# mom-ocean/MOM6

Measured on AMD Instinct MI355X. Metric: simulated-days/wall-sec, higher is better.
Workload: dtype f64

## Files before the change

mom6_amd/csrc/barotropic.hip:

```cpp
#include <algorithm>
#include <type_traits>
#include <vector>
#include <cmath>
#include "mom6x_dev.h"


enum BTW {
  W_q = 0, W_DCor_u, W_DCor_v, W_gtot_E, W_gtot_W, W_gtot_N, W_gtot_S, W_eta, W_eta_PF,
  W_Cor_ref_u, W_Cor_ref_v, W_BT_force_u, W_BT_force_v, W_ubt, W_vbt, W_bt_rem_u, W_bt_rem_v,
  W_uhbt0, W_vhbt0, W_ubt_Cor, W_vbt_Cor, W_uhbt, W_vhbt, W_u_accel_bt, W_v_accel_bt,
  W_eta_src, W_e_anom, W_eta_sum, W_eta_wtd, W_ubt_wtd, W_vbt_wtd, W_eta_pred,
  W_uh0sum, W_vh0sum, W_ubt0, W_vbt0,
  W_f4u, W_f4u_2, W_f4u_3, W_f4u_4, W_f4v, W_f4v_2, W_f4v_3, W_f4v_4,
  W_BTCu,
  W_BTCv = W_BTCu + 10,
  W_BTtmp = W_BTCv + 10,
  W_uhn = W_BTtmp + 12,
  W_vhn,
  W_ubt2, W_vbt2, W_eta_pred2,
  W_COUNT
};

enum BTC { B_FA_EE = 0, B_FA_E0, B_FA_W0, B_FA_WW, B_uBT_WW, B_uBT_EE, B_crvW, B_crvE, B_uh_WW, B_uh_EE };

struct BTState {
  mom6x_barotropic_params P;
  double *frhatu, *frhatv, *IDatu, *IDatv, *ubtav, *vbtav, *eta_cor, *q_D, *D_u_Cor, *D_v_Cor;
  double *work;
  int nstep_last;
  unsigned long long *warn;
  double *warn_info;
  bool la_pending;
  const double *la_pbce;
  double la_underflow;
  bool fr_pending;
  const double *fr_hu, *fr_hv;
};

namespace {

__device__ __forceinline__ double *wp(double *work, const Dm &d, int m) { return work + (size_t)m * d.slab; }

__device__ __forceinline__ double find_uhbt(double u, const double *__restrict__ B, size_t c, size_t slab) {
  if (u == 0.0) return 0.0;
  const double uEE = B[B_uBT_EE * slab + c];
  if (u < uEE) return (u - uEE) * B[B_FA_EE * slab + c] + B[B_uh_EE * slab + c];
  if (u < 0.0) return u * (B[B_FA_E0 * slab + c] + B[B_crvE * slab + c] * (u * u));
  const double uWW = B[B_uBT_WW * slab + c];
  if (u <= uWW) return u * (B[B_FA_W0 * slab + c] + B[B_crvW * slab + c] * (u * u));
  return (u - uWW) * B[B_FA_WW * slab + c] + B[B_uh_WW * slab + c];
}

__global__ void k_bt_init_static(Dm d, const double *__restrict__ G, double Z_to_H, double Mean_SL,
                                 double cor_scale, double H_subroundoff, double *q_D, double *D_u_Cor,
                                 double *D_v_Cor, double *IDatu, double *IDatv) {
  const int i = -1 + blockIdx.x * blockDim.x + threadIdx.x;
  const int j = -1 + blockIdx.y * blockDim.y + threadIdx.y;
  if (i > d.ni - 1 || j > d.nj - 1) return;
  const int st = d.pitch;
  const size_t c = ix2(d, i, j);
  const double *bathyT = gm(G, d, MOM6X_G_bathyT), *areaT = gm(G, d, MOM6X_G_areaT), *mT = gm(G, d, MOM6X_G_mask2dT);
// ... 298 lines not shown
__global__ void k_btcl(Dm d, const double *__restrict__ tmp, double *Bu, double *Bv, int hs) {
  const int i = -hs - 1 + blockIdx.x * blockDim.x + threadIdx.x;
  const int j = -hs - 1 + blockIdx.y * blockDim.y + threadIdx.y;
  if (i > d.ni - 1 + hs || j > d.nj - 1 + hs) return;
  const size_t c = ix2(d, i, j), slab = (size_t)d.slab;
  const double C1_3 = 1.0 / 3.0;
  for (int dir = 0; dir < 2; dir++) {
    if (dir == 0 && j < -hs) continue;
    if (dir == 1 && i < -hs) continue;
    const double *t = tmp + (size_t)(dir * 6) * slab;
    double *B = dir ? Bv : Bu;
    const double FA_EE = t[2 * slab + c], FA_E0 = t[3 * slab + c], FA_W0 = t[4 * slab + c], FA_WW = t[5 * slab + c];
    const double uBT_EE = 1.0 * t[0 * slab + c], uBT_WW = 1.0 * t[1 * slab + c];
    B[B_FA_EE * slab + c] = FA_EE; B[B_FA_E0 * slab + c] = FA_E0; B[B_FA_W0 * slab + c] = FA_W0; B[B_FA_WW * slab + c] = FA_WW;
    B[B_uBT_EE * slab + c] = uBT_EE; B[B_uBT_WW * slab + c] = uBT_WW;
    B[B_uh_EE * slab + c] = uBT_EE * (C1_3 * (2.0 * FA_E0 + FA_EE));
    B[B_uh_WW * slab + c] = uBT_WW * (C1_3 * (2.0 * FA_W0 + FA_WW));
    double crvW = 0.0, crvE = 0.0;
    if (fabs(uBT_WW) > 0.0) crvW = (C1_3 * (FA_WW - FA_W0)) / (uBT_WW * uBT_WW);
    if (fabs(uBT_EE) > 0.0) crvE = (C1_3 * (FA_EE - FA_E0)) / (uBT_EE * uBT_EE);
    B[B_crvW * slab + c] = crvW; B[B_crvE * slab + c] = crvE;
  }
}

__global__ void k_uhbt0(Dm d, const double *__restrict__ work_c, double *work) {
  const int i = -1 + blockIdx.x * blockDim.x + threadIdx.x;
  const int j = -1 + blockIdx.y * blockDim.y + threadIdx.y;
  if (i > d.ni - 1 || j > d.nj - 1) return;
  const size_t c = ix2(d, i, j), slab = (size_t)d.slab;
  if (j >= 0) work[W_uhbt0 * slab + c] = work_c[W_uh0sum * slab + c] - find_uhbt(work_c[W_ubt0 * slab + c], work_c + W_BTCu * slab, c, slab);
  if (i >= 0) work[W_vhbt0 * slab + c] = work_c[W_vh0sum * slab + c] - find_uhbt(work_c[W_vbt0 * slab + c], work_c + W_BTCv * slab, c, slab);
}

__global__ void k_find_Cor(Dm d, double *work, int Sadourny, int isvf, int ievf, int jsvf, int jevf) {
  const int i = isvf - 1 + blockIdx.x * blockDim.x + threadIdx.x;
  const int j = jsvf - 1 + blockIdx.y * blockDim.y + threadIdx.y;
  if (i > ievf + 1 || j > jevf + 1) return;
  const int st = d.pitch;
  const size_t c = ix2(d, i, j), slab = (size_t)d.slab;
  const double *q = work + W_q * slab, *DCor_u = work + W_DCor_u * slab, *DCor_v = work + W_DCor_v * slab;
  double *f4u = work + W_f4u * slab, *f4v = work + W_f4v * slab;
  if (j <= jevf) {
    if (Sadourny) {
      f4v[0 * slab + c] = 1.0 * DCor_u[c - 1] * q[c - 1];
      f4v[1 * slab + c] = 1.0 * DCor_u[c] * q[c];
      f4v[3 * slab + c] = 1.0 * DCor_u[c + st] * q[c];
      f4v[2 * slab + c] = 1.0 * DCor_u[c - 1 + st] * q[c - 1];
    } else {
      f4v[0 * slab + c] = 1.0 * DCor_u[c - 1] * ((q[c] + q[c - 1 - st]) + q[c - 1]) / 3.0;
      f4v[1 * slab + c] = 1.0 * DCor_u[c] * (q[c] + (q[c - 1] + q[c - st])) / 3.0;
      f4v[3 * slab + c] = 1.0 * DCor_u[c + st] * (q[c] + (q[c - 1] + q[c + st])) / 3.0;
      f4v[2 * slab + c] = 1.0 * DCor_u[c - 1 + st] * ((q[c] + q[c - 1 + st]) + q[c - 1]) / 3.0;
    }
  }
  if (i <= ievf) {
    if (Sadourny) {
      f4u[3 * slab + c] = 1.0 * DCor_v[c + 1] * q[c];
      f4u[2 * slab + c] = 1.0 * DCor_v[c] * q[c];
      f4u[0 * slab + c] = 1.0 * DCor_v[c - st] * q[c - st];
      f4u[1 * slab + c] = 1.0 * DCor_v[c + 1 - st] * q[c - st];
    } else {
      f4u[3 * slab + c] = 1.0 * DCor_v[c + 1] * (q[c] + (q[c + 1] + q[c - st])) / 3.0;
      f4u[2 * slab + c] = 1.0 * DCor_v[c] * (q[c] + (q[c - 1] + q[c - st])) / 3.0;
      f4u[0 * slab + c] = 1.0 * DCor_v[c - st] * ((q[c] + q[c - 1 - st]) + q[c - st]) / 3.0;
      f4u[1 * slab + c] = 1.0 * DCor_v[c + 1 - st] * ((q[c] + q[c + 1 - st]) + q[c - st]) / 3.0;
    }
  }
}

__global__ void k_cor_ref_eta_src(Dm d, const double *__restrict__ G, double *work, double *eta_cor, double Instep,
                                  int bound_BT_corr, double maxCFL_Idt, double dt, double Z_to_H, double Z_ref, double maxvel) {
  const int i = -1 + blockIdx.x * blockDim.x + threadIdx.x;
  const int j = -1 + blockIdx.y * blockDim.y + threadIdx.y;
  if (i > d.ni - 1 || j > d.nj - 1) return;
  const int st = d.pitch;
  const size_t c = ix2(d, i, j), slab = (size_t)d.slab;
  const double *f4u = work + W_f4u * slab, *f4v = work + W_f4v * slab;
  const double *ubt_Cor = work + W_ubt_Cor * slab, *vbt_Cor = work + W_vbt_Cor * slab;
  if (j >= 0)
    work[W_Cor_ref_u * slab + c] = (((f4u[3 * slab + c] * vbt_Cor[c + 1]) + (f4u[0 * slab + c] * vbt_Cor[c - st])) +
                                    ((f4u[2 * slab + c] * vbt_Cor[c]) + (f4u[1 * slab + c] * vbt_Cor[c + 1 - st])));
  if (i >= 0)
    work[W_Cor_ref_v * slab + c] = -1.0 * (((f4v[0 * slab + c] * ubt_Cor[c - 1]) + (f4v[3 * slab + c] * ubt_Cor[c + st])) +
                                           ((f4v[1 * slab + c] * ubt_Cor[c]) + (f4v[2 * slab + c] * ubt_Cor[c - 1 + st])));
  if (i >= 0 && j >= 0) {
    const double mT = gm(G, d, MOM6X_G_mask2dT)[c];
    double ec = eta_cor[c];
    if (bound_BT_corr == 2) {
      const double *bathyT = gm(G, d, MOM6X_G_bathyT), *dy_Cu = gm(G, d, MOM6X_G_dy_Cu), *dx_Cv = gm(G, d, MOM6X_G_dx_Cv);
      auto Dat = [&](size_t a, size_t bb, double len) {
        const double H1 = (bathyT[a] + Z_ref) * Z_to_H, H2 = (bathyT[bb] + Z_ref) * Z_to_H;
        double D = 0.0;
        if ((H1 > 0.0) && (H2 > 0.0)) D = len * (2.0 * H1 * H2) / (H1 + H2);
        return D;
      };
      const double DatuW = Dat(c - 1, c, dy_Cu[c - 1]), DatuE = Dat(c, c + 1, dy_Cu[c]);
      const double DatvN = Dat(c, c + st, dx_Cv[c]), DatvS = Dat(c - st, c, dx_Cv[c - st]);
      const double bound = dt * (gm(G, d, MOM6X_G_IareaT)[c] * 0.1 * maxvel * ((DatuW + DatuE) + (DatvN + DatvS)));
      if (fabs(ec) > bound) ec = copysign(bound, ec);
      eta_cor[c] = ec;
    } else if (bound_BT_corr && mT > 0.0) {
      if (ec > 0.0) {
        const double u_max_cor = gm(G, d, MOM6X_G_dxT)[c] * maxCFL_Idt, v_max_cor = gm(G, d, MOM6X_G_dyT)[c] * maxCFL_Idt;
        const double *Bu = work + W_BTCu * slab, *Bv = work + W_BTCv * slab;
        const double *uhbt0 = work + W_uhbt0 * slab, *vhbt0 = work + W_vhbt0 * slab;
        const double eta_cor_max = dt * (gm(G, d, MOM6X_G_IareaT)[c] *
            (((find_uhbt(u_max_cor, Bu, c, slab) + uhbt0[c]) - (find_uhbt(-u_max_cor, Bu, c - 1, slab) + uhbt0[c - 1])) +
             ((find_uhbt(v_max_cor, Bv, c, slab) + vhbt0[c]) - (find_uhbt(-v_max_cor, Bv, c - st, slab) + vhbt0[c - st]))));
        ec = dmin(ec, dmax(0.0, eta_cor_max));
      } else {
        const double Htot = gm(G, d, MOM6X_G_bathyT)[c] * Z_to_H + work[W_eta * slab + c];
        ec = dmax(ec, -dmax(0.0, Htot));
      }
      eta_cor[c] = ec;
    }
    work[W_eta_src * slab + c] = mT * (Instep * ec);
  }
}

__global__ void k_bt_copy_in(Dm d, double *work, const double *__restrict__ eta_in, const double *__restrict__ eta_PF_in,
                             const double *__restrict__ q_D, const double *__restrict__ D_u_Cor,
                             const double *__restrict__ D_v_Cor) {
  const int i = -d.halo - 1 + blockIdx.x * blockDim.x + threadIdx.x;
  const int j = -d.halo - 1 + blockIdx.y * blockDim.y + threadIdx.y;
  if (i > d.ni - 1 + d.halo || j > d.nj - 1 + d.halo) return;
  const size_t c = ix2(d, i, j), slab = (size_t)d.slab;
  if (i >= -d.halo && j >= -d.halo) { work[W_eta * slab + c] = eta_in[c]; work[W_eta_PF * slab + c] = eta_PF_in[c]; }
  work[W_q * slab + c] = q_D[c]; work[W_DCor_u * slab + c] = D_u_Cor[c]; work[W_DCor_v * slab + c] = D_v_Cor[c];
}

struct LoopArgs {
  double dtbt, dgeo_de, vel_underflow, trans_wt1, trans_wt2;
  double wt_accel, wt_trans, wt_vel, wt_eta, wt_accel2;
  int project, bracket_bug, find_etaav;
  int f4_on_the_fly, Sadourny;
  int store_uhn, have_uhn;
  int pred_next;
  double wt_accel2_next;
  int isv, iev, jsv, jev;
};

__global__ void __launch_bounds__(256)
k_bt_pred(Dm d, const double *__restrict__ G, double *work, LoopArgs A, int p_ubt, int p_vbt, int p_pred, int sel) {
  const int i = I_BASE(A.isv - 1) + blockIdx.x * blockDim.x + threadIdx.x;
  const int j = A.jsv - 1 + blockIdx.y * blockDim.y + threadIdx.y;
  if (i < A.isv - 1 || i > A.iev + 1 || j > A.jev + 1) return;
  if (sel) { const bool own = (i >= 0 && i <= d.ni - 1 && j >= 0 && j <= d.nj - 1); if (own != (sel == 1)) return; }
  const int st = d.pitch;
  const size_t c = ix2(d, i, j), slab = (size_t)d.slab;
  double eta_PF_BT;
  if (A.project) {
    eta_PF_BT = work[W_eta * slab + c];
  } else {
    const double *ubt = work + (size_t)p_ubt * slab, *vbt = work + (size_t)p_vbt * slab;
    const double *Bu = work + W_BTCu * slab, *Bv = work + W_BTCv * slab;
    const double *uhbt0 = work + W_uhbt0 * slab, *vhbt0 = work + W_vhbt0 * slab;
    double uW, uE, vS, vN;
    if (A.have_uhn) {
      const double *uhn = work + W_uhn * slab, *vhn = work + W_vhn * slab;
      uW = uhn[c - 1]; uE = uhn[c]; vS = vhn[c - st]; vN = vhn[c];
    } else {
      uW = find_uhbt(ubt[c - 1], Bu, c - 1, slab) + uhbt0[c - 1];
      uE = find_uhbt(ubt[c], Bu, c, slab) + uhbt0[c];
      vS = find_uhbt(vbt[c - st], Bv, c - st, slab) + vhbt0[c - st];
      vN = find_uhbt(vbt[c], Bv, c, slab) + vhbt0[c];
    }
    eta_PF_BT = (work[W_eta * slab + c] + work[W_eta_src * slab + c]) +
                (A.dtbt * gm(G, d, MOM6X_G_IareaT)[c]) * ((uW - uE) + (vS - vN));
    work[(size_t)p_pred * slab + c] = eta_PF_BT;
  }
  if (A.find_etaav && (fabs(A.wt_accel2) > 0.0) && i >= 0 && i <= d.ni - 1 && j >= 0 && j <= d.nj - 1)
    work[W_eta_sum * slab + c] = work[W_eta_sum * slab + c] + A.wt_accel2 * eta_PF_BT;
}

__device__ __forceinline__ void f4u_of(const double *__restrict__ q, const double *__restrict__ DCor_v, size_t c, int st, int Sadourny,
                                       double &f0, double &f1, double &f2, double &f3) {
  if (Sadourny) {
    f3 = 1.0 * DCor_v[c + 1] * q[c];
    f2 = 1.0 * DCor_v[c] * q[c];
    f0 = 1.0 * DCor_v[c - st] * q[c - st];
    f1 = 1.0 * DCor_v[c + 1 - st] * q[c - st];
  } else {
    f3 = 1.0 * DCor_v[c + 1] * (q[c] + (q[c + 1] + q[c - st])) / 3.0;
    f2 = 1.0 * DCor_v[c] * (q[c] + (q[c - 1] + q[c - st])) / 3.0;
    f0 = 1.0 * DCor_v[c - st] * ((q[c] + q[c - 1 - st]) + q[c - st]) / 3.0;
    f1 = 1.0 * DCor_v[c + 1 - st] * ((q[c] + q[c + 1 - st]) + q[c - st]) / 3.0;
  }
}
__device__ __forceinline__ void f4v_of(const double *__restrict__ q, const double *__restrict__ DCor_u, size_t c, int st, int Sadourny,
                                       double &f0, double &f1, double &f2, double &f3) {
  if (Sadourny) {
    f0 = 1.0 * DCor_u[c - 1] * q[c - 1];
    f1 = 1.0 * DCor_u[c] * q[c];
    f3 = 1.0 * DCor_u[c + st] * q[c];
    f2 = 1.0 * DCor_u[c - 1 + st] * q[c - 1];
  } else {
    f0 = 1.0 * DCor_u[c - 1] * ((q[c] + q[c - 1 - st]) + q[c - 1]) / 3.0;
    f1 = 1.0 * DCor_u[c] * (q[c] + (q[c - 1] + q[c - st])) / 3.0;
    f3 = 1.0 * DCor_u[c + st] * (q[c] + (q[c - 1] + q[c + st])) / 3.0;
    f2 = 1.0 * DCor_u[c - 1 + st] * ((q[c] + q[c - 1 + st]) + q[c - 1]) / 3.0;
  }
}

template <int DIR>
__device__ __forceinline__ void bt_face_update(const Dm &d, const double *__restrict__ G, const double *work, const LoopArgs &A, size_t c, int st,
                                               size_t slab, const double *etaB, double vel, double n0, double n1, double n2, double n3,
                                               int bracket_bug, double &newv, double &CorPF) {
  const double *eta_PF = work + W_eta_PF * slab;
  double Cor, PF, f0, f1, f2, f3;
  if (DIR == 0) {
    const double *gE = work + W_gtot_E * slab, *gW = work + W_gtot_W * slab;
    PF = (((etaB[c] - eta_PF[c]) * gE[c]) - ((etaB[c + 1] - eta_PF[c + 1]) * gW[c + 1])) * A.dgeo_de * gm(G, d, MOM6X_G_IdxCu)[c];
    f4u_of(work + W_q * slab, work + W_DCor_v * slab, c, st, A.Sadourny, f0, f1, f2, f3);
    Cor = (((f3 * n0) + (f0 * n1)) + ((f2 * n2) + (f1 * n3))) - work[W_Cor_ref_u * slab + c];
    newv = work[W_bt_rem_u * slab + c] * (vel + A.dtbt * ((work[W_BT_force_u * slab + c] + Cor) + PF));
  } else {
    const double *gN = work + W_gtot_N * slab, *gS = work + W_gtot_S * slab;
    PF = (((etaB[c] - eta_PF[c]) * gN[c]) - ((etaB[c + st] - eta_PF[c + st]) * gS[c + st])) * A.dgeo_de * gm(G, d, MOM6X_G_IdyCv)[c];
    f4v_of(work + W_q * slab, work + W_DCor_u * slab, c, st, A.Sadourny, f0, f1, f2, f3);
    if (bracket_bug) Cor = -1.0 * (((f0 * n0) + (f1 * n1)) + ((f3 * n2) + (f2 * n3))) - work[W_Cor_ref_v * slab + c];
    else Cor = -1.0 * (((f0 * n0) + (f3 * n2)) + ((f1 * n1) + (f2 * n3))) - work[W_Cor_ref_v * slab + c];
    newv = work[W_bt_rem_v * slab + c] * (vel + A.dtbt * ((work[W_BT_force_v * slab + c] + Cor) + PF));
  }
  if (fabs(newv) < A.vel_underflow) newv = 0.0;
  CorPF = Cor + PF;
}

template <int DIR>
__global__ void __launch_bounds__(256)
k_bt_vel(Dm d, const double *__restrict__ G, double *work, double *btav, double *hbtav, LoopArgs A,
         int a0, int a1, int b0, int b1, int bracket_bug) {
  const int i = I_BASE(a0) + blockIdx.x * blockDim.x + threadIdx.x;
  const int j = b0 + blockIdx.y * blockDim.y + threadIdx.y;
  if (i < a0 || i > a1 || j > b1) return;
// ... 294 lines not shown
bool barotropic_ready(const mom6x_ctx *c) { return c->bts != nullptr; }

void bt_state_free(mom6x_ctx *c) {
  if (!c->bts) return;
  BTState *s = c->bts;
  double *ptrs[] = { s->frhatu, s->frhatv, s->IDatu, s->IDatv, s->ubtav, s->vbtav, s->eta_cor, s->q_D, s->D_u_Cor,
                     s->D_v_Cor, s->work, s->warn_info };
  for (double *p : ptrs) (void)hipFree(p);
  (void)hipFree(s->warn);
  delete s;
  c->bts = nullptr;
}

extern "C" int mom6x_btstep_warnings(mom6x_ctx *c, int reset, long long *count, double *info) {
  REQUIRE(c && c->bts && count, MOM6X_EINVAL, "mom6x_btstep_warnings: barotropic_init has not been called");
  HIPCHK(hipSetDevice(c->device));
  HIPCHK(hipStreamSynchronize(c->stream));
  unsigned long long w[2];
  HIPCHK(hipMemcpy(w, c->bts->warn, sizeof(w), hipMemcpyDeviceToHost));
  *count = (long long)w[0];
  if (info) HIPCHK(hipMemcpy(info, c->bts->warn_info, 4 * sizeof(double), hipMemcpyDeviceToHost));
  if (reset) HIPCHK(hipMemset(c->bts->warn, 0, sizeof(w)));
  return MOM6X_OK;
}

static int bt_state_alloc(mom6x_ctx *c, BTState *s) {
  const Dm d = c->d;
  const size_t n2 = (size_t)d.slab, n3 = n2 * d.nk;
  double **p3[] = { &s->frhatu, &s->frhatv };
  for (double **q : p3) { HIPCHK(hipMalloc(q, n3 * sizeof(double))); HIPCHK(hipMemsetAsync(*q, 0, n3 * sizeof(double), c->stream)); }
  double **p2[] = { &s->IDatu, &s->IDatv, &s->ubtav, &s->vbtav, &s->eta_cor, &s->q_D, &s->D_u_Cor, &s->D_v_Cor };
  for (double **q : p2) { HIPCHK(hipMalloc(q, n2 * sizeof(double))); HIPCHK(hipMemsetAsync(*q, 0, n2 * sizeof(double), c->stream)); }
  HIPCHK(hipMalloc(&s->work, (size_t)W_COUNT * n2 * sizeof(double)));
  HIPCHK(hipMalloc(&s->warn, 2 * sizeof(unsigned long long))); HIPCHK(hipMemsetAsync(s->warn, 0, 2 * sizeof(unsigned long long), c->stream));
  HIPCHK(hipMalloc(&s->warn_info, 4 * sizeof(double))); HIPCHK(hipMemsetAsync(s->warn_info, 0, 4 * sizeof(double), c->stream));
  return MOM6X_OK;
}

extern "C" int mom6x_barotropic_init(mom6x_ctx *c, const mom6x_barotropic_params *p) {
  REQUIRE(c && p, MOM6X_EINVAL, "mom6x_barotropic_init: null argument");
  REQUIRE(p->bt_thick_scheme >= MOM6X_BT_THICK_FROM_BT_CONT && p->bt_thick_scheme <= MOM6X_BT_THICK_ARITHMETIC, MOM6X_EINVAL,
          "barotropic_init: Unrecognized setting of BT_THICK_SCHEME");
  REQUIRE(c->dims.halo >= 2, MOM6X_EINVAL, "barotropic: halo >= 2 required");
  REQUIRE(p->BTHALO <= c->dims.halo, MOM6X_EINVAL,
          "barotropic_init: BTHALO exceeds the halo of the tile context; create the context with halo = max(NIHALO, BTHALO)");
  REQUIRE(p->min_stencil >= 0 && p->min_stencil <= c->dims.halo, MOM6X_EINVAL, "barotropic_init: bad BT_WIDE_HALO_MIN_STENCIL");
  HIPCHK(hipSetDevice(c->device));
  const Dm d = c->d;
  if (!c->bts) {
    c->bts = new BTState();
    if (const int rc = bt_state_alloc(c, c->bts)) { bt_state_free(c); return rc; }
  }
  BTState *s = c->bts;
  s->P = *p;
  s->nstep_last = 0;
  const dim3 b = blk2();
  KLAUNCH(c, "k_bt_init_static", k_bt_init_static, grid3(d.ni + 1, d.nj + 1, 1, b), b, d, c->G, c->GV.Z_to_H, p->Z_ref,
                     p->BT_Coriolis_scale, c->GV.H_subroundoff, s->q_D, s->D_u_Cor, s->D_v_Cor, s->IDatu, s->IDatv);
  double *f[] = { s->q_D, s->D_u_Cor, s->D_v_Cor };
  const int stg[] = { 3, 1, 2 }, nks[] = { 1, 1, 1 };
  halo_wrap(c, f, stg, nks, 3);
  HIPCHK(hipGetLastError());
  return MOM6X_OK;
}

extern "C" double *mom6x_barotropic_field(mom6x_ctx *c, int which) {
  if (!c || !c->bts) return nullptr;
  BTState *s = c->bts;
  if ((which == 3 || which == 4) && bt_frhat_materialize(c)) return nullptr;
  switch (which) {
    case 0: return s->ubtav; case 1: return s->vbtav; case 2: return s->eta_cor; case 3: return s->frhatu;
    case 4: return s->frhatv; case 5: return s->IDatu; case 6: return s->IDatv; case 7: return s->q_D;
    case 8: return s->D_u_Cor; case 9: return s->D_v_Cor; case 10: return s->work;
    default: return nullptr;
  }
}

extern "C" int mom6x_barotropic_dtbt(mom6x_ctx *c, double *get, const double *set) {
  REQUIRE(c && c->bts, MOM6X_EINVAL, "mom6x_barotropic_dtbt: Module MOM_barotropic must be initialized before it is used.");
  if (set) { REQUIRE(*set > 0.0, MOM6X_EINVAL, "mom6x_barotropic_dtbt: DTBT must be positive"); c->bts->P.dtbt = *set; }
  if (get) *get = c->bts->P.dtbt;
  return MOM6X_OK;
}

extern "C" int mom6x_btcalc_strict(mom6x_ctx *c, const double *h, const double *h_u, const double *h_v) {
  REQUIRE(c && c->bts, MOM6X_EINVAL, "btcalc: Module MOM_barotropic must be initialized before it is used.");
  REQUIRE((h_u && h_v) || c->bts->P.bt_thick_scheme != MOM6X_BT_THICK_FROM_BT_CONT, MOM6X_EINVAL,
// ... 107 lines not shown
                      const double *taux_bot, const double *tauy_bot, const double *uh0, const double *vh0, const double *u_uh0,
                      const double *v_vh0, double *etaav, bool defer_layer_accel) {
  REQUIRE(c && c->bts, MOM6X_EINVAL, "btstep: Module MOM_barotropic must be initialized before it is used.");
  REQUIRE(U_in && V_in && eta_in && bc_accel_u && bc_accel_v && taux && tauy && pbce && eta_PF_in && U_Cor && V_Cor &&
          accel_layer_u && accel_layer_v && eta_out && uhbtav && vhbtav && visc_rem_u && visc_rem_v,
          MOM6X_EINVAL, "btstep: null mandatory array");
  const bool add_uh0 = (uh0 != nullptr);
  REQUIRE(!add_uh0 || (vh0 && u_uh0 && v_vh0), MOM6X_EINVAL,
          "btstep: vh0, u_uh0, and v_vh0 must be associated if uh0 is used.");
  REQUIRE((taux_bot != nullptr) == (tauy_bot != nullptr), MOM6X_EINVAL, "btstep: taux_bot and tauy_bot come together");
  HIPCHK(hipSetDevice(c->device));
  const Dm d = c->d;
  const mom6x_barotropic_params &P = c->bts->P;
  BTState *s = c->bts;
  double *work = s->work;
  const size_t slab = (size_t)d.slab;
  const dim3 b = blk2();
  hipStream_t st = c->stream;
  const int is = 0, ie = d.ni - 1, js = 0, je = d.nj - 1;

  const double Idt = 1.0 / dt;
  const bool evolving_face_areas = !BT_cont && P.nonlinear_continuity && P.nonlin_cont_update_period > 0;
  const int stencil = evolving_face_areas ? std::max(2, P.min_stencil) : ((P.min_stencil > 1) ? P.min_stencil : 1);
  const int num_cycles = (P.use_wide_halos && d.halo / stencil >= 1) ? d.halo / stencil : 1;
  const int isvf = is - (num_cycles - 1) * stencil, ievf = ie + (num_cycles - 1) * stencil;
  const int jsvf = js - (num_cycles - 1) * stencil, jevf = je + (num_cycles - 1) * stencil;
  REQUIRE(P.dtbt > 0.0, MOM6X_EINVAL, "btstep: dtbt must be positive (call set_dtbt or set params.dtbt)");
  const int nstep = (int)ceil(dt / P.dtbt - 0.0001);
  s->nstep_last = nstep;
  const double Instep = 1.0 / (double)nstep;
  const double dtbt = dt * Instep;
  const double dgeo_de = 1.0 + P.G_extra;

  HIPCHK(hipMemsetAsync(work, 0, (size_t)W_COUNT * slab * sizeof(double), st));
  KLAUNCH(c, "k_bt_copy_in", k_bt_copy_in, grid3(d.ni + 2 * d.halo + 1, d.nj + 2 * d.halo + 1, 1, b), b, d, work, eta_in,
                     eta_PF_in, s->q_D, s->D_u_Cor, s->D_v_Cor);

  ColArgs Au;
  memset(&Au, 0, sizeof(Au));
  Au.visc_rem = visc_rem_u; Au.frhat = s->frhatu; Au.U_Cor = U_Cor; Au.pbce = pbce; Au.uh0 = uh0; Au.u_uh0 = u_uh0;
  Au.U_in = U_in; Au.bc_accel = bc_accel_u; Au.tau = taux; Au.tau_bot = taux_bot; Au.IDat = s->IDatu;
  Au.ubt_Cor = work + W_ubt_Cor * slab; Au.gtot_m = work + W_gtot_E * slab; Au.gtot_p = work + W_gtot_W * slab;
  Au.uh0sum = work + W_uh0sum * slab; Au.ubt0 = work + W_ubt0 * slab; Au.ubt = work + W_ubt * slab;
  Au.BT_force = work + W_BT_force_u * slab; Au.bt_rem = work + W_bt_rem_u * slab;
  Au.Instep = Instep; Au.RZ_to_H = c->GV.RZ_to_H; Au.vel_underflow = P.vel_underflow; Au.nstep = nstep;
  Au.wt_uv_bug = P.wt_uv_bug; Au.visc_rem_u_uh0 = P.visc_rem_u_uh0; Au.strong_drag = P.strong_drag;
  ColArgs Av = Au;
  Av.visc_rem = visc_rem_v; Av.frhat = s->frhatv; Av.U_Cor = V_Cor; Av.uh0 = vh0; Av.u_uh0 = v_vh0; Av.U_in = V_in;
  Av.bc_accel = bc_accel_v; Av.tau = tauy; Av.tau_bot = tauy_bot; Av.IDat = s->IDatv;
  Av.ubt_Cor = work + W_vbt_Cor * slab; Av.gtot_m = work + W_gtot_N * slab; Av.gtot_p = work + W_gtot_S * slab;
  Av.uh0sum = work + W_vh0sum * slab; Av.ubt0 = work + W_vbt0 * slab; Av.ubt = work + W_vbt * slab;
  Av.BT_force = work + W_BT_force_v * slab; Av.bt_rem = work + W_bt_rem_v * slab;
  if (s->fr_pending) {
    Au.hf = s->fr_hu; Av.hf = s->fr_hv; Au.h_neglect = Av.h_neglect = c->GV.H_subroundoff;
    KLAUNCH(c, "k_bt_col<0>", (k_bt_col<0, true>), grid3(nxa(d.ni + 1, -1), d.nj, 1, b), b, d, c->G, Au);
    KLAUNCH(c, "k_bt_col<1>", (k_bt_col<1, true>), grid3(d.ni, d.nj + 1, 1, b), b, d, c->G, Av);
  } else {
    { const int rcm = bt_frhat_materialize(c); if (rcm) return rcm; }
    KLAUNCH(c, "k_bt_col<0>", (k_bt_col<0, false>), grid3(nxa(d.ni + 1, -1), d.nj, 1, b), b, d, c->G, Au);
    KLAUNCH(c, "k_bt_col<1>", (k_bt_col<1, false>), grid3(d.ni, d.nj + 1, 1, b), b, d, c->G, Av);
  }

  double *tmp = work + W_BTtmp * slab;
  if (BT_cont) KLAUNCH(c, "k_btcont_copy", k_btcont_copy, grid3(d.ni + 1, d.nj + 1, 1, b), b, d, *BT_cont, tmp);
  else KLAUNCH(c, "k_face_areas_as_fits", k_face_areas_as_fits, grid3(d.ni + 3, d.nj + 3, 1, b), b, d, c->G, P.Z_ref, c->GV.Z_to_H, tmp,
               P.nonlinear_continuity ? (const double *)(work + W_eta * slab) : (const double *)nullptr);
  {
    double *f[18]; int stg[18], nks[18];
    for (int m = 0; m < 12; m++) { f[m] = tmp + (size_t)m * slab; stg[m] = (m < 6) ? 1 : 2; nks[m] = 1; }
    double *g[] = { work + W_gtot_E * slab, work + W_gtot_N * slab, work + W_gtot_W * slab, work + W_gtot_S * slab,
                    work + W_ubt_Cor * slab, work + W_vbt_Cor * slab };
    const int gs[] = { 0, 0, 0, 0, 1, 2 };
    for (int m = 0; m < 6; m++) { f[12 + m] = g[m]; stg[12 + m] = gs[m]; nks[12 + m] = 1; }
    halo_wrap(c, f, stg, nks, 18);
  }
  const int hs = 1 + ievf - ie;
  KLAUNCH(c, "k_btcl", k_btcl, grid3(d.ni + 2 * hs + 1, d.nj + 2 * hs + 1, 1, b), b, d, tmp, work + W_BTCu * slab,
                     work + W_BTCv * slab, hs);
  if (add_uh0) KLAUNCH(c, "k_uhbt0", k_uhbt0, grid3(d.ni + 1, d.nj + 1, 1, b), b, d, work, work);

  KLAUNCH(c, "k_find_Cor", k_find_Cor, grid3(ievf - isvf + 3, jevf - jsvf + 3, 1, b), b, d, work, P.Sadourny, isvf, ievf, jsvf, jevf);
  KLAUNCH(c, "k_cor_ref_eta_src", k_cor_ref_eta_src, grid3(d.ni + 1, d.nj + 1, 1, b), b, d, c->G, work, s->eta_cor, Instep,
                     P.bound_BT_corr ? ((BT_cont && P.BT_cont_bounds) ? 1 : 2) : 0, P.maxCFL_BT_cont * Idt, dt, c->GV.Z_to_H, P.Z_ref, P.maxvel);
  {
    std::vector<double *> f = { work + W_eta_PF * slab, work + W_eta_src * slab, work + W_bt_rem_u * slab, work + W_bt_rem_v * slab,
                                work + W_BT_force_u * slab, work + W_BT_force_v * slab };
    std::vector<int> stg = { 0, 0, 1, 2, 1, 2 };
    if (add_uh0) { f.push_back(work + W_uhbt0 * slab); stg.push_back(1); f.push_back(work + W_vhbt0 * slab); stg.push_back(2); }
    f.push_back(work + W_Cor_ref_u * slab); stg.push_back(1); f.push_back(work + W_Cor_ref_v * slab); stg.push_back(2);
    std::vector<int> nks(f.size(), 1);
    halo_wrap(c, f.data(), stg.data(), nks.data(), (int)f.size());
  }

  double dt_filt;
  if (P.dt_bt_filter >= 0.0) dt_filt = 0.5 * fmax(0.0, fmin(P.dt_bt_filter, 2.0 * dt));
  else dt_filt = 0.5 * fmax(0.0, dt * fmin(-P.dt_bt_filter, 2.0));
  const int nfilter = (int)ceil(dt_filt / dtbt);
  const int nt = nstep + nfilter;
  REQUIRE(nt > 0, MOM6X_EINVAL, "btstep: number of barotropic step (nstep+nfilter) is 0");
  std::vector<double> wt_vel(nt + 2, 0.0), wt_eta(nt + 2, 0.0), wt_trans(nt + 2, 0.0), wt_accel(nt + 2, 0.0), wt_accel2(nt + 2, 0.0);
  double sum_wt_vel = 0.0, sum_wt_eta = 0.0, sum_wt_accel = 0.0, sum_wt_trans = 0.0;
  for (int n = 1; n <= nt; n++) {
    if ((n == nstep) || (dt_filt - abs(n - nstep) * dtbt >= 0.0)) { wt_vel[n] = 1.0; wt_eta[n] = 1.0; }
    else if (dtbt + dt_filt - abs(n - nstep) * dtbt > 0.0) { wt_vel[n] = 1.0 + (dt_filt / dtbt) - abs(n - nstep); wt_eta[n] = wt_vel[n]; }
    else { wt_vel[n] = 0.0; wt_eta[n] = 0.0; }
    sum_wt_vel = sum_wt_vel + wt_vel[n]; sum_wt_eta = sum_wt_eta + wt_eta[n];
  }
  for (int n = nt; n >= 1; n--) {
    wt_trans[n] = wt_trans[n + 1] + wt_eta[n];
    wt_accel[n] = wt_accel[n + 1] + wt_vel[n];
    sum_wt_accel = sum_wt_accel + wt_accel[n]; sum_wt_trans = sum_wt_trans + wt_trans[n];
  }
  const double I_sum_wt_vel = 1.0 / sum_wt_vel, I_sum_wt_accel = 1.0 / sum_wt_accel;
  const double I_sum_wt_eta = 1.0 / sum_wt_eta, I_sum_wt_trans = 1.0 / sum_wt_trans;
  for (int n = 1; n <= nt; n++) {
    wt_vel[n] = wt_vel[n] * I_sum_wt_vel;
    wt_accel2[n] = wt_accel[n] * I_sum_wt_accel;
    wt_trans[n] = wt_trans[n] * I_sum_wt_trans;
    wt_accel[n] = wt_accel[n] * I_sum_wt_accel;
    wt_eta[n] = wt_eta[n] * I_sum_wt_eta;
  }

  HIPCHK(hipMemsetAsync(s->ubtav, 0, slab * sizeof(double), st));
  HIPCHK(hipMemsetAsync(s->vbtav, 0, slab * sizeof(double), st));
  HIPCHK(hipMemsetAsync(uhbtav, 0, slab * sizeof(double), st));
  HIPCHK(hipMemsetAsync(vhbtav, 0, slab * sizeof(double), st));
  LoopArgs L;
  memset(&L, 0, sizeof(L));
  L.dtbt = dtbt; L.dgeo_de = dgeo_de; L.vel_underflow = P.vel_underflow;
  if (P.BT_project_velocity) { L.trans_wt1 = (1.0 + P.bebt); L.trans_wt2 = -P.bebt; }
  else { L.trans_wt1 = P.bebt; L.trans_wt2 = (1.0 - P.bebt); }
  L.project = P.BT_project_velocity; L.find_etaav = (etaav != nullptr);
  L.f4_on_the_fly = 1; L.Sadourny = P.Sadourny;
  int isv = is, iev = ie, jsv = js, jev = je;
  const bool pass_uhn = !P.clip_velocity && !P.BT_project_velocity && !evolving_face_areas;
  L.store_uhn = pass_uhn ? 1 : 0;
  static const int substep_env = [] { const char *e = getenv("MOM6X_BT_SUBSTEP"); return !e ? 0 : (!strcmp(e, "kernels") ? 1 : (!strcmp(e, "fused") ? 2 : 0)); }();
  const bool small_tile = ((long)d.ni * d.nj <= 512L * 1024L);
  const bool fused = pass_uhn && (substep_env == 2 || (substep_env == 0 && small_tile));
  const bool overlap_loop = fused && c->bt_overlap && halo_can_overlap(c) && d.ni >= 96 && d.nj >= 32;
  SubPlanes SP = { W_ubt, fused ? W_ubt2 : W_ubt, W_vbt, fused ? W_vbt2 : W_vbt, W_eta_pred, fused ? W_eta_pred2 : W_eta_pred };
  const int loop_stg[] = { 0, 1, 2, 1, 2 }, loop_nk[] = { 1, 1, 1, 1, 1 };
  bool pred_done = false;
  for (int n = 1; n <= nt; n++) {
    if (P.clip_velocity)
      KLAUNCH(c, "k_bt_clip", k_bt_clip, grid3(iev - isv + 2, jev - jsv + 2, 1, b), b, d, c->G, work, dt, P.CFL_trunc, isv, iev, jsv, jev);
    L.have_uhn = (pass_uhn && n > 1) ? 1 : 0;
    bool travelling = false;
    if ((iev - stencil < ie) || (jev - stencil < je)) {
      double *loop_f[] = { work + W_eta * slab, work + (size_t)SP.u_in * slab, work + (size_t)SP.v_in * slab, work + W_uhn * slab,
                           work + W_vhn * slab };
      if (overlap_loop) travelling = halo_start_packed(c, loop_f, loop_stg, loop_nk, (pass_uhn && n > 1) ? 5 : 3);
      else halo_wrap(c, loop_f, loop_stg, loop_nk, (pass_uhn && n > 1) ? 5 : 3);
      isv = isvf; iev = ievf; jsv = jsvf; jev = jevf;
    } else {
      isv += stencil; iev -= stencil; jsv += stencil; jev -= stencil;
    }
    if (evolving_face_areas && n > 1 && ((n - 1) % P.nonlin_cont_update_period == 0))
      KLAUNCH(c, "k_face_areas_eta", k_face_areas_eta, grid3(iev - isv + 4, jev - jsv + 4, 1, b), b, d, c->G, c->GV.Z_to_H,
              (const double *)(work + W_eta * slab), work + W_BTCu * slab, work + W_BTCv * slab, isv, iev, jsv, jev);
    L.isv = isv; L.iev = iev; L.jsv = jsv; L.jev = jev;
    L.wt_accel = wt_accel[n]; L.wt_trans = wt_trans[n]; L.wt_vel = wt_vel[n]; L.wt_eta = wt_eta[n]; L.wt_accel2 = wt_accel2[n];
    const bool do_pred = (!P.BT_project_velocity || L.find_etaav) && !pred_done;
    if (do_pred)
      KLAUNCH(c, "k_bt_pred", k_bt_pred, grid3(nxa(iev - isv + 3, isv - 1), jev - jsv + 3, 1, b), b, d, c->G, work, L, SP.u_in, SP.v_in, SP.e_in,
              travelling ? 1 : 0);
    pred_done = pass_uhn && n < nt && !((iev - stencil < ie) || (jev - stencil < je));
    L.pred_next = pred_done ? 1 : 0;
    L.wt_accel2_next = pred_done ? wt_accel2[n + 1] : 0.0;
    const bool v_first = (((n + c->first_direction) % 2) == 1);
    if (fused) {
#define SUBSTEP(BX, BY, SEL) do {                                                                                                     \
      const int OX = v_first ? BX - 2 : BX - 1, OY = v_first ? BY - 1 : BY - 2;                                                        \
// ... 56 lines not shown
```

Measured before the change: 0.1928.

## Shrink per-call barotropic workspace clearing and fold Coriolis factors into consumer

Reorders the barotropic work planes so those that must start at zero each call sit in a leading block. When a signature of parameters, step count, halo and path flags matches the previous call, only that block is memset instead of the whole workspace. The separate f4u/f4v precompute kernel and its eight planes are removed, and k_cor_ref_eta_src computes the factors inline. Four small memsets are replaced with one zeroing kernel. The risk is correctness: the remaining planes must be fully overwritten before they are read, or stale values from the previous call leak into the new one.

Result: no change. 0.1926 (-0.1%).

```diff
diff --git a/mom6_amd/csrc/barotropic.hip b/mom6_amd/csrc/barotropic.hip
--- a/mom6_amd/csrc/barotropic.hip
+++ b/mom6_amd/csrc/barotropic.hip
@@ -6,27 +6,51 @@
 
 
 enum BTW {
-  W_q = 0, W_DCor_u, W_DCor_v, W_gtot_E, W_gtot_W, W_gtot_N, W_gtot_S, W_eta, W_eta_PF,
-  W_Cor_ref_u, W_Cor_ref_v, W_BT_force_u, W_BT_force_v, W_ubt, W_vbt, W_bt_rem_u, W_bt_rem_v,
-  W_uhbt0, W_vhbt0, W_ubt_Cor, W_vbt_Cor, W_uhbt, W_vhbt, W_u_accel_bt, W_v_accel_bt,
-  W_eta_src, W_e_anom, W_eta_sum, W_eta_wtd, W_ubt_wtd, W_vbt_wtd, W_eta_pred,
+  W_eta = 0,
+  W_eta_pred,
+  W_eta_pred2,
+  W_ubt, W_vbt,
+  W_ubt2, W_vbt2,
+  W_uhn, W_vhn,
+  W_uhbt, W_vhbt,
+  W_u_accel_bt, W_v_accel_bt,
+  W_eta_sum,
+  W_eta_wtd,
+  W_ubt_wtd, W_vbt_wtd,
+  W_CLEAR_END,
+  W_q = W_CLEAR_END, W_DCor_u, W_DCor_v,
+  W_eta_PF,
+  W_gtot_E, W_gtot_N,
+  W_gtot_W, W_gtot_S,
+  W_ubt_Cor, W_vbt_Cor,
+  W_BT_force_u, W_BT_force_v,
+  W_bt_rem_u, W_bt_rem_v,
   W_uh0sum, W_vh0sum, W_ubt0, W_vbt0,
-  W_f4u, W_f4u_2, W_f4u_3, W_f4u_4, W_f4v, W_f4v_2, W_f4v_3, W_f4v_4,
+  W_uhbt0, W_vhbt0,
+  W_Cor_ref_u, W_Cor_ref_v,
+  W_eta_src,
+  W_e_anom,
   W_BTCu,
   W_BTCv = W_BTCu + 10,
   W_BTtmp = W_BTCv + 10,
-  W_uhn = W_BTtmp + 12,
-  W_vhn,
-  W_ubt2, W_vbt2, W_eta_pred2,
-  W_COUNT
+  W_COUNT = W_BTtmp + 12
 };
 
 enum BTC { B_FA_EE = 0, B_FA_E0, B_FA_W0, B_FA_WW, B_uBT_WW, B_uBT_EE, B_crvW, B_crvE, B_uh_WW, B_uh_EE };
+
+struct BTSig {
+  bool valid;
+  mom6x_barotropic_params P;
+  int nstep, halo;
+  unsigned shape;
+  const void *comm;
+};
 
 struct BTState {
   mom6x_barotropic_params P;
   double *frhatu, *frhatv, *IDatu, *IDatv, *ubtav, *vbtav, *eta_cor, *q_D, *D_u_Cor, *D_v_Cor;
   double *work;
+  BTSig sig;
   int nstep_last;
   unsigned long long *warn;
   double *warn_info;
@@ -391,57 +415,53 @@
   if (i >= 0) work[W_vhbt0 * slab + c] = work_c[W_vh0sum * slab + c] - find_uhbt(work_c[W_vbt0 * slab + c], work_c + W_BTCv * slab, c, slab);
 }
 
-__global__ void k_find_Cor(Dm d, double *work, int Sadourny, int isvf, int ievf, int jsvf, int jevf) {
-  const int i = isvf - 1 + blockIdx.x * blockDim.x + threadIdx.x;
-  const int j = jsvf - 1 + blockIdx.y * blockDim.y + threadIdx.y;
-  if (i > ievf + 1 || j > jevf + 1) return;
-  const int st = d.pitch;
-  const size_t c = ix2(d, i, j), slab = (size_t)d.slab;
-  const double *q = work + W_q * slab, *DCor_u = work + W_DCor_u * slab, *DCor_v = work + W_DCor_v * slab;
-  double *f4u = work + W_f4u * slab, *f4v = work + W_f4v * slab;
-  if (j <= jevf) {
-    if (Sadourny) {
-      f4v[0 * slab + c] = 1.0 * DCor_u[c - 1] * q[c - 1];
-      f4v[1 * slab + c] = 1.0 * DCor_u[c] * q[c];
-      f4v[3 * slab + c] = 1.0 * DCor_u[c + st] * q[c];
-      f4v[2 * slab + c] = 1.0 * DCor_u[c - 1 + st] * q[c - 1];
-    } else {
-      f4v[0 * slab + c] = 1.0 * DCor_u[c - 1] * ((q[c] + q[c - 1 - st]) + q[c - 1]) / 3.0;
-      f4v[1 * slab + c] = 1.0 * DCor_u[c] * (q[c] + (q[c - 1] + q[c - st])) / 3.0;
-      f4v[3 * slab + c] = 1.0 * DCor_u[c + st] * (q[c] + (q[c - 1] + q[c + st])) / 3.0;
-      f4v[2 * slab + c] = 1.0 * DCor_u[c - 1 + st] * ((q[c] + q[c - 1 + st]) + q[c - 1]) / 3.0;
-    }
-  }
-  if (i <= ievf) {
-    if (Sadourny) {
-      f4u[3 * slab + c] = 1.0 * DCor_v[c + 1] * q[c];
-      f4u[2 * slab + c] = 1.0 * DCor_v[c] * q[c];
-      f4u[0 * slab + c] = 1.0 * DCor_v[c - st] * q[c - st];
-      f4u[1 * slab + c] = 1.0 * DCor_v[c + 1 - st] * q[c - st];
-    } else {
-      f4u[3 * slab + c] = 1.0 * DCor_v[c + 1] * (q[c] + (q[c + 1] + q[c - st])) / 3.0;
-      f4u[2 * slab + c] = 1.0 * DCor_v[c] * (q[c] + (q[c - 1] + q[c - st])) / 3.0;
-      f4u[0 * slab + c] = 1.0 * DCor_v[c - st] * ((q[c] + q[c - 1 - st]) + q[c - st]) / 3.0;
-      f4u[1 * slab + c] = 1.0 * DCor_v[c + 1 - st] * ((q[c] + q[c + 1 - st]) + q[c - st]) / 3.0;
-    }
-  }
-}
-
-__global__ void k_cor_ref_eta_src(Dm d, const double *__restrict__ G, double *work, double *eta_cor, double Instep,
+__device__ __forceinline__ void f4u_of(const double *__restrict__ q, const double *__restrict__ DCor_v, size_t c, int st, int Sadourny,
+                                       double &f0, double &f1, double &f2, double &f3) {
+  if (Sadourny) {
+    f3 = 1.0 * DCor_v[c + 1] * q[c];
+    f2 = 1.0 * DCor_v[c] * q[c];
+    f0 = 1.0 * DCor_v[c - st] * q[c - st];
+    f1 = 1.0 * DCor_v[c + 1 - st] * q[c - st];
+  } else {
+    f3 = 1.0 * DCor_v[c + 1] * (q[c] + (q[c + 1] + q[c - st])) / 3.0;
+    f2 = 1.0 * DCor_v[c] * (q[c] + (q[c - 1] + q[c - st])) / 3.0;
+    f0 = 1.0 * DCor_v[c - st] * ((q[c] + q[c - 1 - st]) + q[c - st]) / 3.0;
+    f1 = 1.0 * DCor_v[c + 1 - st] * ((q[c] + q[c + 1 - st]) + q[c - st]) / 3.0;
+  }
+}
+__device__ __forceinline__ void f4v_of(const double *__restrict__ q, const double *__restrict__ DCor_u, size_t c, int st, int Sadourny,
+                                       double &f0, double &f1, double &f2, double &f3) {
+  if (Sadourny) {
+    f0 = 1.0 * DCor_u[c - 1] * q[c - 1];
+    f1 = 1.0 * DCor_u[c] * q[c];
+    f3 = 1.0 * DCor_u[c + st] * q[c];
+    f2 = 1.0 * DCor_u[c - 1 + st] * q[c - 1];
+  } else {
+    f0 = 1.0 * DCor_u[c - 1] * ((q[c] + q[c - 1 - st]) + q[c - 1]) / 3.0;
+    f1 = 1.0 * DCor_u[c] * (q[c] + (q[c - 1] + q[c - st])) / 3.0;
+    f3 = 1.0 * DCor_u[c + st] * (q[c] + (q[c - 1] + q[c + st])) / 3.0;
+    f2 = 1.0 * DCor_u[c - 1 + st] * ((q[c] + q[c - 1 + st]) + q[c - 1]) / 3.0;
+  }
+}
+
+__global__ void k_cor_ref_eta_src(Dm d, const double *__restrict__ G, double *work, double *eta_cor, double Instep, int Sadourny,
                                   int bound_BT_corr, double maxCFL_Idt, double dt, double Z_to_H, double Z_ref, double maxvel) {
   const int i = -1 + blockIdx.x * blockDim.x + threadIdx.x;
   const int j = -1 + blockIdx.y * blockDim.y + threadIdx.y;
   if (i > d.ni - 1 || j > d.nj - 1) return;
   const int st = d.pitch;
   const size_t c = ix2(d, i, j), slab = (size_t)d.slab;
-  const double *f4u = work + W_f4u * slab, *f4v = work + W_f4v * slab;
+  const double *q = work + W_q * slab;
   const double *ubt_Cor = work + W_ubt_Cor * slab, *vbt_Cor = work + W_vbt_Cor * slab;
-  if (j >= 0)
-    work[W_Cor_ref_u * slab + c] = (((f4u[3 * slab + c] * vbt_Cor[c + 1]) + (f4u[0 * slab + c] * vbt_Cor[c - st])) +
-                                    ((f4u[2 * slab + c] * vbt_Cor[c]) + (f4u[1 * slab + c] * vbt_Cor[c + 1 - st])));
-  if (i >= 0)
-    work[W_Cor_ref_v * slab + c] = -1.0 * (((f4v[0 * slab + c] * ubt_Cor[c - 1]) + (f4v[3 * slab + c] * ubt_Cor[c + st])) +
-                                           ((f4v[1 * slab + c] * ubt_Cor[c]) + (f4v[2 * slab + c] * ubt_Cor[c - 1 + st])));
+  double f0, f1, f2, f3;
+  if (j >= 0) {
+    f4u_of(q, work + W_DCor_v * slab, c, st, Sadourny, f0, f1, f2, f3);
+    work[W_Cor_ref_u * slab + c] = (((f3 * vbt_Cor[c + 1]) + (f0 * vbt_Cor[c - st])) + ((f2 * vbt_Cor[c]) + (f1 * vbt_Cor[c + 1 - st])));
+  }
+  if (i >= 0) {
+    f4v_of(q, work + W_DCor_u * slab, c, st, Sadourny, f0, f1, f2, f3);
+    work[W_Cor_ref_v * slab + c] = -1.0 * (((f0 * ubt_Cor[c - 1]) + (f3 * ubt_Cor[c + st])) + ((f1 * ubt_Cor[c]) + (f2 * ubt_Cor[c - 1 + st])));
+  }
   if (i >= 0 && j >= 0) {
     const double mT = gm(G, d, MOM6X_G_mask2dT)[c];
     double ec = eta_cor[c];
@@ -488,11 +508,18 @@
   work[W_q * slab + c] = q_D[c]; work[W_DCor_u * slab + c] = D_u_Cor[c]; work[W_DCor_v * slab + c] = D_v_Cor[c];
 }
 
+__global__ void __launch_bounds__(256)
+k_bt_zero_means(size_t n, double *ubtav, double *vbtav, double *uhbtav, double *vhbtav) {
+  const size_t t = (size_t)blockIdx.x * blockDim.x + threadIdx.x;
+  if (t >= n) return;
+  ubtav[t] = 0.0; vbtav[t] = 0.0; uhbtav[t] = 0.0; vhbtav[t] = 0.0;
+}
+
 struct LoopArgs {
   double dtbt, dgeo_de, vel_underflow, trans_wt1, trans_wt2;
   double wt_accel, wt_trans, wt_vel, wt_eta, wt_accel2;
   int project, bracket_bug, find_etaav;
-  int f4_on_the_fly, Sadourny;
+  int Sadourny;
   int store_uhn, have_uhn;
   int pred_next;
   double wt_accel2_next;
@@ -530,35 +557,6 @@
   }
   if (A.find_etaav && (fabs(A.wt_accel2) > 0.0) && i >= 0 && i <= d.ni - 1 && j >= 0 && j <= d.nj - 1)
     work[W_eta_sum * slab + c] = work[W_eta_sum * slab + c] + A.wt_accel2 * eta_PF_BT;
-}
-
-__device__ __forceinline__ void f4u_of(const double *__restrict__ q, const double *__restrict__ DCor_v, size_t c, int st, int Sadourny,
-                                       double &f0, double &f1, double &f2, double &f3) {
-  if (Sadourny) {
-    f3 = 1.0 * DCor_v[c + 1] * q[c];
-    f2 = 1.0 * DCor_v[c] * q[c];
-    f0 = 1.0 * DCor_v[c - st] * q[c - st];
-    f1 = 1.0 * DCor_v[c + 1 - st] * q[c - st];
-  } else {
-    f3 = 1.0 * DCor_v[c + 1] * (q[c] + (q[c + 1] + q[c - st])) / 3.0;
-    f2 = 1.0 * DCor_v[c] * (q[c] + (q[c - 1] + q[c - st])) / 3.0;
-    f0 = 1.0 * DCor_v[c - st] * ((q[c] + q[c - 1 - st]) + q[c - st]) / 3.0;
-    f1 = 1.0 * DCor_v[c + 1 - st] * ((q[c] + q[c + 1 - st]) + q[c - st]) / 3.0;
-  }
-}
-__device__ __forceinline__ void f4v_of(const double *__restrict__ q, const double *__restrict__ DCor_u, size_t c, int st, int Sadourny,
-                                       double &f0, double &f1, double &f2, double &f3) {
-  if (Sadourny) {
-    f0 = 1.0 * DCor_u[c - 1] * q[c - 1];
-    f1 = 1.0 * DCor_u[c] * q[c];
-    f3 = 1.0 * DCor_u[c + st] * q[c];
-    f2 = 1.0 * DCor_u[c - 1 + st] * q[c - 1];
-  } else {
-    f0 = 1.0 * DCor_u[c - 1] * ((q[c] + q[c - 1 - st]) + q[c - 1]) / 3.0;
-    f1 = 1.0 * DCor_u[c] * (q[c] + (q[c - 1] + q[c - st])) / 3.0;
-    f3 = 1.0 * DCor_u[c + st] * (q[c] + (q[c - 1] + q[c + st])) / 3.0;
-    f2 = 1.0 * DCor_u[c - 1 + st] * ((q[c] + q[c - 1 + st]) + q[c - 1]) / 3.0;
-  }
 }
 
 template <int DIR>
@@ -919,6 +917,7 @@
   double **p2[] = { &s->IDatu, &s->IDatv, &s->ubtav, &s->vbtav, &s->eta_cor, &s->q_D, &s->D_u_Cor, &s->D_v_Cor };
   for (double **q : p2) { HIPCHK(hipMalloc(q, n2 * sizeof(double))); HIPCHK(hipMemsetAsync(*q, 0, n2 * sizeof(double), c->stream)); }
   HIPCHK(hipMalloc(&s->work, (size_t)W_COUNT * n2 * sizeof(double)));
+  HIPCHK(hipMemsetAsync(s->work, 0, (size_t)W_COUNT * n2 * sizeof(double), c->stream));
   HIPCHK(hipMalloc(&s->warn, 2 * sizeof(unsigned long long))); HIPCHK(hipMemsetAsync(s->warn, 0, 2 * sizeof(unsigned long long), c->stream));
   HIPCHK(hipMalloc(&s->warn_info, 4 * sizeof(double))); HIPCHK(hipMemsetAsync(s->warn_info, 0, 4 * sizeof(double), c->stream));
   return MOM6X_OK;
@@ -940,6 +939,7 @@
   }
   BTState *s = c->bts;
   s->P = *p;
+  s->sig.valid = false;
   s->nstep_last = 0;
   const dim3 b = blk2();
   KLAUNCH(c, "k_bt_init_static", k_bt_init_static, grid3(d.ni + 1, d.nj + 1, 1, b), b, d, c->G, c->GV.Z_to_H, p->Z_ref,
@@ -1113,7 +1113,25 @@
   const double dtbt = dt * Instep;
   const double dgeo_de = 1.0 + P.G_extra;
 
-  HIPCHK(hipMemsetAsync(work, 0, (size_t)W_COUNT * slab * sizeof(double), st));
+  const bool pass_uhn = !P.clip_velocity && !P.BT_project_velocity && !evolving_face_areas;
+  static const int substep_env = [] { const char *e = getenv("MOM6X_BT_SUBSTEP"); return !e ? 0 : (!strcmp(e, "kernels") ? 1 : (!strcmp(e, "fused") ? 2 : 0)); }();
+  const bool small_tile = ((long)d.ni * d.nj <= 512L * 1024L);
+  const bool fused = pass_uhn && (substep_env == 2 || (substep_env == 0 && small_tile));
+  const bool overlap_loop = fused && c->bt_overlap && halo_can_overlap(c) && d.ni >= 96 && d.nj >= 32;
+
+  {
+    BTSig sig;
+    memset(&sig, 0, sizeof(sig));
+    sig.valid = true;
+    memcpy(&sig.P, &s->P, sizeof(sig.P)); sig.P.dtbt = 0.0;
+    sig.nstep = nstep; sig.halo = d.halo; sig.comm = (const void *)c->comm;
+    sig.shape = (BT_cont ? 1u : 0u) | (add_uh0 ? 2u : 0u) | (taux_bot ? 4u : 0u) | (s->fr_pending ? 8u : 0u) | (fused ? 16u : 0u) |
+                (overlap_loop ? 32u : 0u);
+    const bool same = s->sig.valid && !memcmp(&sig.P, &s->sig.P, sizeof(sig.P)) && sig.nstep == s->sig.nstep && sig.halo == s->sig.halo &&
+                      sig.shape == s->sig.shape && sig.comm == s->sig.comm;
+    s->sig = sig;
+    HIPCHK(hipMemsetAsync(work, 0, (size_t)(same ? W_CLEAR_END : W_COUNT) * slab * sizeof(double), st));
+  }
   KLAUNCH(c, "k_bt_copy_in", k_bt_copy_in, grid3(d.ni + 2 * d.halo + 1, d.nj + 2 * d.halo + 1, 1, b), b, d, work, eta_in,
                      eta_PF_in, s->q_D, s->D_u_Cor, s->D_v_Cor);
 
@@ -1160,8 +1178,7 @@
                      work + W_BTCv * slab, hs);
   if (add_uh0) KLAUNCH(c, "k_uhbt0", k_uhbt0, grid3(d.ni + 1, d.nj + 1, 1, b), b, d, work, work);
 
-  KLAUNCH(c, "k_find_Cor", k_find_Cor, grid3(ievf - isvf + 3, jevf - jsvf + 3, 1, b), b, d, work, P.Sadourny, isvf, ievf, jsvf, jevf);
-  KLAUNCH(c, "k_cor_ref_eta_src", k_cor_ref_eta_src, grid3(d.ni + 1, d.nj + 1, 1, b), b, d, c->G, work, s->eta_cor, Instep,
+  KLAUNCH(c, "k_cor_ref_eta_src", k_cor_ref_eta_src, grid3(d.ni + 1, d.nj + 1, 1, b), b, d, c->G, work, s->eta_cor, Instep, P.Sadourny,
                      P.bound_BT_corr ? ((BT_cont && P.BT_cont_bounds) ? 1 : 2) : 0, P.maxCFL_BT_cont * Idt, dt, c->GV.Z_to_H, P.Z_ref, P.maxvel);
   {
     std::vector<double *> f = { work + W_eta_PF * slab, work + W_eta_src * slab, work + W_bt_rem_u * slab, work + W_bt_rem_v * slab,
@@ -1202,24 +1219,16 @@
     wt_eta[n] = wt_eta[n] * I_sum_wt_eta;
   }
 
-  HIPCHK(hipMemsetAsync(s->ubtav, 0, slab * sizeof(double), st));
-  HIPCHK(hipMemsetAsync(s->vbtav, 0, slab * sizeof(double), st));
-  HIPCHK(hipMemsetAsync(uhbtav, 0, slab * sizeof(double), st));
-  HIPCHK(hipMemsetAsync(vhbtav, 0, slab * sizeof(double), st));
+  KLAUNCH(c, "k_bt_zero_means", k_bt_zero_means, dim3((unsigned)((slab + 255) / 256)), dim3(256), slab, s->ubtav, s->vbtav, uhbtav, vhbtav);
   LoopArgs L;
   memset(&L, 0, sizeof(L));
   L.dtbt = dtbt; L.dgeo_de = dgeo_de; L.vel_underflow = P.vel_underflow;
   if (P.BT_project_velocity) { L.trans_wt1 = (1.0 + P.bebt); L.trans_wt2 = -P.bebt; }
   else { L.trans_wt1 = P.bebt; L.trans_wt2 = (1.0 - P.bebt); }
   L.project = P.BT_project_velocity; L.find_etaav = (etaav != nullptr);
-  L.f4_on_the_fly = 1; L.Sadourny = P.Sadourny;
+  L.Sadourny = P.Sadourny;
   int isv = is, iev = ie, jsv = js, jev = je;
-  const bool pass_uhn = !P.clip_velocity && !P.BT_project_velocity && !evolving_face_areas;
   L.store_uhn = pass_uhn ? 1 : 0;
-  static const int substep_env = [] { const char *e = getenv("MOM6X_BT_SUBSTEP"); return !e ? 0 : (!strcmp(e, "kernels") ? 1 : (!strcmp(e, "fused") ? 2 : 0)); }();
-  const bool small_tile = ((long)d.ni * d.nj <= 512L * 1024L);
-  const bool fused = pass_uhn && (substep_env == 2 || (substep_env == 0 && small_tile));
-  const bool overlap_loop = fused && c->bt_overlap && halo_can_overlap(c) && d.ni >= 96 && d.nj >= 32;
   SubPlanes SP = { W_ubt, fused ? W_ubt2 : W_ubt, W_vbt, fused ? W_vbt2 : W_vbt, W_eta_pred, fused ? W_eta_pred2 : W_eta_pred };
   const int loop_stg[] = { 0, 1, 2, 1, 2 }, loop_nk[] = { 1, 1, 1, 1, 1 };
   bool pred_done = false;
```
